# psklavos1/NeRF-Sys

Hardware: AMD Instinct MI355X
Metric: rays/sec (train step) + full-image PSNR, 800×800 Lego, 64+128 samples (higher is better)
Workload: dtype f32; 1 GPU; Lego-style 800x800 (synthetic analytic scene, 100 views), 64 coarse + 128 fine hierarchical, 2 x (8x256 MLP), fp32, train step incl. ray gen + Adam [fused engine]; global_batch=4096, rays_per_gpu=4096, parallelism=dp1, precision=fp32, fp32_gemm=split, full=False

## Files before the change

### include/nerf_amd.h

```cpp
#ifndef NERF_AMD_H
#define NERF_AMD_H

#include <stdint.h>
#include <stddef.h>
#include <hip/hip_runtime_api.h>

#ifdef __cplusplus
extern "C" {
#endif

#define NERF_OK 0
#define NERF_E_ARG (-1)
#define NERF_E_ALIGN (-2)
#define NERF_E_ENUM (-3)
#define NERF_E_WORKSPACE (-4)
#define NERF_E_UNSUPPORTED (-5)


int nerf_rays_gen(const float* c2w, int n_poses, const int32_t* pix, int64_t n, int H, int W,
                  float fx, float fy, float cx, float cy, int center_pixels, float near_v, float far_v,
                  const float* aabb, float aabb_max_bound, float aabb_invalid,
                  const uint8_t* images_u8, float* rays_out, float* rgb_out, hipStream_t stream);

int nerf_pick_pixels(int64_t n, int n_images, int H, int W, uint64_t seed, int32_t* pix_out,
                     hipStream_t stream);

int nerf_pick_pixels_dseed(int64_t n, int n_images, int H, int W, uint64_t seed_base, uint64_t seed_mul,
                           const int64_t* step_dev, int32_t* pix_out, hipStream_t stream);

int nerf_clamp_near_far(float* rays, int64_t n, int has_near, float near_v, int has_far, float far_v,
                        float eps, float invalid_value, uint8_t* valid_out, hipStream_t stream);

int nerf_rays_ndc(const float* rays_in, int64_t n, int H, int W, float focal, float near_plane,
                  float* rays_out, hipStream_t stream);


int nerf_sample_stratified(const float* rays, int64_t n, int S, int randomized, const float* u,
                           uint64_t seed, float* t_out, hipStream_t stream);

int nerf_build_xd(const float* rays, const float* t, int64_t n, int S, float* xd_out, hipStream_t stream);

int nerf_sample_pdf(const float* t, const float* w, int64_t n, int S, int n_imp, const float* u, int det,
                    uint64_t seed, float* t_out, hipStream_t stream);


int nerf_freq_encode(const float* x, int64_t n, int D, int L, int include_input, float* out, int ld_out,
                     hipStream_t stream);


int64_t nerf_mlp_layout(int64_t* table);

int64_t nerf_mlp_workspace_bytes(int64_t M, int training);

int nerf_mlp_fwd(const float* w, const float* x_d, int64_t M, float* rgb_sigma, void* ws, int64_t ws_bytes,
                 int training, hipEvent_t* events, hipStream_t stream);


int nerf_mlp_bwd(const float* w, int64_t M, const float* d_rgb_sigma, float* d_w, int accumulate, void* ws,
                 int64_t ws_bytes, hipEvent_t* events, hipStream_t stream);

int64_t nerf_mlp_workspace_bytes_2s(int64_t M);
int nerf_mlp_bwd_2s(const float* w, int64_t M, const float* d_rgb_sigma, float* d_w, int accumulate, void* ws,
                    int64_t ws_bytes, hipEvent_t* events, hipStream_t stream, hipStream_t wgrad_stream, hipEvent_t* sync);

#define NERF_MLP_NATIVE_FP32 1
#define NERF_MLP_NATIVE_DGRAD 2
int nerf_mlp_fwd_ex(const float* w, const float* x_d, int64_t M, float* rgb_sigma, void* ws, int64_t ws_bytes,
                    int training, int flags, hipEvent_t* events, hipStream_t stream);
int nerf_mlp_bwd_ex(const float* w, int64_t M, const float* d_rgb_sigma, float* d_w, int accumulate, void* ws,
                    int64_t ws_bytes, int flags, hipEvent_t* events, hipStream_t stream);
int nerf_mlp_bwd_2s_ex(const float* w, int64_t M, const float* d_rgb_sigma, float* d_w, int accumulate, void* ws,
                       int64_t ws_bytes, int flags, hipEvent_t* events, hipStream_t stream, hipStream_t wgrad_stream,
                       hipEvent_t* sync);

#define NERF_BF16_LAYERED_FWD 1
#define NERF_BF16_LAYERED_BWD 2
int64_t nerf_mlp_workspace_bytes_bf16(int64_t M, int training);
int nerf_mlp_fwd_bf16(const float* w, const float* x_d, int64_t M, float* rgb_sigma, void* ws, int64_t ws_bytes,
                      int training, int flags, hipEvent_t* events, hipStream_t stream);
int nerf_mlp_bwd_bf16(const float* w, int64_t M, const float* d_rgb_sigma, float* d_w, int accumulate, void* ws,
                      int64_t ws_bytes, int flags, hipEvent_t* events, hipStream_t stream);

int64_t nerf_mlp_workspace_bytes_f16(int64_t M, int training);
int nerf_mlp_fwd_f16(const float* w, const float* x_d, int64_t M, float* rgb_sigma, void* ws, int64_t ws_bytes,
                     int training, int flags, hipEvent_t* events, hipStream_t stream);
int nerf_mlp_bwd_f16(const float* w, int64_t M, const float* d_rgb_sigma, float* d_w, int accumulate, void* ws,
                     int64_t ws_bytes, int flags, hipEvent_t* events, hipStream_t stream);


int nerf_composite_fwd(const float* rgb_sigma, const float* t, const float* bg, int64_t n, int S,
                       float sigma_scale, float* rgb, float* depth, float* weights, float* acc,
                       const float* gt, int color_space, float inv_count, float* loss_sum, float* d_rgb,
                       hipStream_t stream);

int nerf_composite_bwd(const float* rgb_sigma, const float* t, const float* bg, int64_t n, int S,
                       float sigma_scale, const float* g_rgb, const float* g_depth, const float* g_acc,
                       const float* g_weights, float* d_rgb_sigma, hipStream_t stream);


int nerf_grad_sqnorm(const float* g, int64_t n, float* partials, hipStream_t stream);

int nerf_adam(float* p, const float* g, float* m, float* v, int64_t n, const int64_t* seg_off_host,
              const double* seg_lr_host, int n_seg, double beta1, double beta2, float eps, float weight_decay,
              int step, const float* partials, float max_norm, hipStream_t stream);

int nerf_adam_dstep(float* p, const float* g, float* m, float* v, int64_t n, const int64_t* seg_off_host,
                    const double* seg_lr_host, int n_seg, double beta1, double beta2, float eps, float weight_decay,
                    const int64_t* step_dev, const float* partials, float max_norm, hipStream_t stream);


#define NERF_HASH_MAX_LEVELS 32

typedef struct {
  int32_t levels;
  int32_t features_per_level;
  int32_t log2_hashmap_size;
  int32_t interpolation;
  int32_t resolutions[NERF_HASH_MAX_LEVELS];
} NerfHashGrid;
// ... 194 lines not shown
```

### nerf-sys_amd/csrc/gemm_x6.hpp

```cpp
#pragma once
#include "gemm_bf16.hpp"

typedef float x6_f32x2 __attribute__((ext_vector_type(2)));
typedef __bf16 x6_bf16x2 __attribute__((ext_vector_type(2)));
typedef float x6_f32x4 __attribute__((ext_vector_type(4)));
__device__ __forceinline__ uint32_t x6_pack(float a, float b) {
  return __builtin_bit_cast(uint32_t, __builtin_convertvector(x6_f32x2{a, b}, x6_bf16x2));
}

__device__ __forceinline__ void x6_split4(const float4 v, uint2& h, uint2& m, uint2& l) {
  const uint32_t h0 = x6_pack(v.x, v.y), h1 = x6_pack(v.z, v.w);
  const float r0 = v.x - nerf_bf16_lo(h0), r1 = v.y - nerf_bf16_hi(h0);
  const float r2 = v.z - nerf_bf16_lo(h1), r3 = v.w - nerf_bf16_hi(h1);
  const uint32_t m0 = x6_pack(r0, r1), m1 = x6_pack(r2, r3);
  const uint32_t l0 = x6_pack(r0 - nerf_bf16_lo(m0), r1 - nerf_bf16_hi(m0));
  const uint32_t l1 = x6_pack(r2 - nerf_bf16_lo(m1), r3 - nerf_bf16_hi(m1));
  h = make_uint2(h0, h1);
  m = make_uint2(m0, m1);
  l = make_uint2(l0, l1);
}

__device__ constexpr int X6_PA[6] = {2, 1, 0, 1, 0, 0};
__device__ constexpr int X6_PB[6] = {0, 1, 2, 0, 1, 0};
#define X6_MFMA_BLOCK(acc_, TM_, TN_, FIRST_, SECOND_)                                                      \
  _Pragma("unroll") for (int t_ = 0; t_ < 6; ++t_)                                                        \
    _Pragma("unroll") for (int a_ = 0; a_ < TM_; ++a_)                                                    \
      _Pragma("unroll") for (int b_ = 0; b_ < TN_; ++b_)                                                  \
        acc_[a_][b_] = __builtin_amdgcn_mfma_f32_32x32x16_bf16(FIRST_, SECOND_, acc_[a_][b_], 0, 0, 0);

struct X6Job {
  const float* src;
  nerf_bf16* dst;
  int rows, cols, lds, transpose;
  int64_t plane;
};
struct X6Jobs {
  X6Job j[16];
};
static __global__ void x6_planes_kernel(X6Jobs jobs) {
  const X6Job J = jobs.j[blockIdx.z];
  __shared__ float tile[32][33];
  const int r0 = blockIdx.y * 32, c0 = blockIdx.x * 32;
  if (r0 >= J.rows || c0 >= J.cols) return;
  const int tx = threadIdx.x & 31, ty = threadIdx.x >> 5;
  for (int y = ty; y < 32; y += 8) {
    const int r = r0 + y, c = c0 + tx;
    tile[y][tx] = (r < J.rows && c < J.cols) ? J.src[(int64_t)r * J.lds + c] : 0.f;
  }
  __syncthreads();
  for (int y = ty; y < 32; y += 8) {
    const float v = J.transpose ? tile[tx][y] : tile[y][tx];
    const int orow = J.transpose ? c0 + y : r0 + y, ocol = J.transpose ? r0 + tx : c0 + tx;
    const int orows = J.transpose ? J.cols : J.rows, ocols = J.transpose ? J.rows : J.cols;
    if (orow < orows && ocol < ocols) {
      const nerf_bf16 h = (nerf_bf16)v;
      const float r1 = v - (float)h;
      const nerf_bf16 m = (nerf_bf16)r1;
      const nerf_bf16 l = (nerf_bf16)(r1 - (float)m);
      const int64_t o = (int64_t)orow * ocols + ocol;
      J.dst[o] = h;
      J.dst[J.plane + o] = m;
      J.dst[2 * J.plane + o] = l;
    }
  }
}


constexpr int X6E_PITCH = 36;
constexpr int X6E_WAVE_FLOATS = 32 * X6E_PITCH;
template <int TM, int TN, int EPI>
__device__ __forceinline__ void x6_epilogue_lds(nerf_f32x16 (&acc)[TM][TN], int64_t mw, int n0, int lane,
                                                const float* __restrict__ bias, float* __restrict__ C, int ldc,
                                                const uint32_t* __restrict__ mbits, int ldmb,
                                                uint32_t* __restrict__ mbits_out, float* E) {
  const int li = lane & 31, lh = lane >> 5;
  const int rr = lane >> 3, cc = 4 * (lane & 7);
#pragma unroll
  for (int b = 0; b < TN; ++b) {
    const int nb = n0 + b * 32;
    const int g = nb >> 5;
    float4 bv[4];
#pragma unroll
    for (int q = 0; q < 4; ++q) {
      bv[q] = make_float4(0.f, 0.f, 0.f, 0.f);
      if (EPI == EPI_BIAS || EPI == EPI_BIAS_RELU) bv[q] = *reinterpret_cast<const float4*>(bias + nb + 8 * q + 4 * lh);
    }
#pragma unroll
    for (int a = 0; a < TM; ++a) {
      const int64_t m = mw + a * 32 + li;
      uint32_t word = 0;
      if (EPI == EPI_MASK) word = mbits[m * ldmb + g];
#pragma unroll
      for (int q = 0; q < 4; ++q) {
        float v[4];
#pragma unroll
        for (int e = 0; e < 4; ++e) {
          v[e] = acc[a][b][4 * q + e];
          const float bb = e == 0 ? bv[q].x : (e == 1 ? bv[q].y : (e == 2 ? bv[q].z : bv[q].w));
          if (EPI == EPI_BIAS) v[e] += bb;
          if (EPI == EPI_BIAS_RELU) {
            v[e] = fmaxf(v[e] + bb, 0.f);
            word |= (v[e] > 0.f ? 1u : 0u) << (8 * q + 4 * lh + e);
          }
          if (EPI == EPI_MASK) v[e] = ((word >> (8 * q + 4 * lh + e)) & 1u) ? v[e] : 0.f;
        }
        *reinterpret_cast<float4*>(E + li * X6E_PITCH + 8 * q + 4 * lh) = make_float4(v[0], v[1], v[2], v[3]);
      }
      if (EPI == EPI_BIAS_RELU && mbits_out) {
        word |= __shfl_xor(word, 32, 64);
        if (lh == 0) mbits_out[m * ldmb + g] = word;
      }
      float4 o[4];
#pragma unroll
      for (int i = 0; i < 4; ++i) o[i] = *reinterpret_cast<const float4*>(E + (rr + 8 * i) * X6E_PITCH + cc);
#pragma unroll
      for (int i = 0; i < 4; ++i)
        *reinterpret_cast<float4*>(C + (mw + a * 32 + rr + 8 * i) * ldc + nb + cc) = o[i];
    }
  }
}

template <int EPI, bool BIGSMALL, int NKC, int TN>
__global__ __launch_bounds__(512, 1) void gemm_nt_x6w_kernel(const float* __restrict__ A, int lda,
                                                             const nerf_bf16* __restrict__ Bp, int ldb, int64_t bplane,
                                                             const float* __restrict__ bias, float* __restrict__ C,
                                                             int ldc, const uint32_t* __restrict__ mbits, int ldmb,
                                                             uint32_t* __restrict__ mbits_out, int K, int n_ntiles) {
  constexpr int BK = 32, NW = 8, TM = 1;
  constexpr int WTM = 32 * TM, BM = WTM * NW, BN = 32 * TN;
  constexpr int KS = BK / 16;
  constexpr int LS = BK;
  static_assert(BK == 32, "the swizzle assumes four 16-B chunks per row");
  auto sw = [](int r, int q) { return q ^ ((r >> 2) & 3); };
  constexpr int PL = BN * LS;
  static_assert(2 * 3 * PL >= NW * X6E_WAVE_FLOATS * 2, "epilogue tiles");
  __shared__ __attribute__((aligned(16))) nerf_bf16 smem[2 * 3 * PL];

  const int tile = xcd_remap(blockIdx.x, gridDim.x);
  const int mt = tile / n_ntiles, nt = tile - mt * n_ntiles;
  const int64_t m0 = (int64_t)mt * BM;
  const int n0 = nt * BN;
  const int tid = threadIdx.x, lane = tid & 63, wave = tid >> 6;
  const int li = lane & 31, lh = lane >> 5;
  const nerf_bf16* Bb = Bp + (int64_t)n0 * ldb;
  const float* At = A + (m0 + wave * WTM) * lda;
  int aoff[TM];
#pragma unroll
  for (int a = 0; a < TM; ++a) aoff[a] = (a * 32 + li) * lda + 8 * lh;

  constexpr bool A3 = NKC > 0;
  float4 ra[A3 ? 3 : 2][TM][KS][2];
  constexpr int GPP = BN * BK * 2 / 1024, GPW = 3 * GPP / NW;
  static_assert(GPW * NW == 3 * GPP && GPP * 1024 == BN * BK * 2, "weight staging");
  const int wave_u = __builtin_amdgcn_readfirstlane(tid >> 6);
  const uint32_t gofs = (uint32_t)((((lane >> 2) * ldb) + 8 * ((lane & 3) ^ ((lane >> 4) & 3))) * 2);
  const uint32_t smem_u32 = (uint32_t)(uintptr_t)(const __attribute__((address_space(3))) char*)smem;
#define X6W_ALOAD(set_, k0_)                                                                              \
  _Pragma("unroll") for (int a = 0; a < TM; ++a)                                                         \
    _Pragma("unroll") for (int ks = 0; ks < KS; ++ks)                                                    \
      _Pragma("unroll") for (int hf = 0; hf < 2; ++hf)                                                   \
        ra[set_][a][ks][hf] = *reinterpret_cast<const float4*>(At + aoff[a] + (k0_) + 16 * ks + 4 * hf);
  constexpr int BPG = 2;
#define X6W_BLOAD(k0_, dbuf_)                                                                             \
  {                                                                                                       \
    _Pragma("unroll") for (int a = 0; a < TM; ++a)                                                       \
      _Pragma("unroll") for (int ks = 0; ks < KS; ++ks)                                                  \
        asm volatile("" ::"v"(__builtin_bit_cast(x6_f32x4, ra[j][a][ks][0])),                            \
                     "v"(__builtin_bit_cast(x6_f32x4, ra[j][a][ks][1])) : "memory");                     \
    _Pragma("unroll") for (int i = 0; i < GPW; ++i) {                                                    \
      const int g_ = wave_u + NW * i, p_ = g_ / GPP, rb_ = (g_ % GPP) * 16;                              \
      const nerf_bf16* sb_ = Bb + p_ * bplane + (int64_t)rb_ * ldb + (k0_);                              \
      const uint32_t dst_ = smem_u32 + (uint32_t)((((dbuf_) * 3 + p_) * PL + rb_ * LS) * 2);             \
      unsigned keep_;                                                                                     \
      asm volatile("s_mov_b32 %0, m0\n\ts_mov_b32 m0, %3\n\ts_nop 0\n\tglobal_load_lds_dwordx4 %1, %2\n\t" \
                   "s_mov_b32 m0, %0" : "=&s"(keep_) : "v"(gofs), "s"(sb_), "s"(dst_) : "memory");       \
    }                                                                                                     \
  }
  static_assert(TM * KS * 2 == 4, "vmcnt: the activation loads after the weight DMA");
#define X6W_BWAIT() asm volatile("s_waitcnt vmcnt(4)" ::: "memory")

  nerf_f32x16 acc[TM][TN], accs[BIGSMALL ? TM : 1][BIGSMALL ? TN : 1];
#pragma unroll
  for (int a = 0; a < TM; ++a)
#pragma unroll
    for (int b = 0; b < TN; ++b)
#pragma unroll
      for (int r = 0; r < 16; ++r) {
        acc[a][b][r] = 0.f;
        if constexpr (BIGSMALL) accs[a][b][r] = 0.f;
      }

  const int nk = A3 ? NKC : K / BK;
  X6W_ALOAD(0, 0);
  X6W_ALOAD(1, (nk > 1 ? 1 : 0) * BK);
  {
    const int j = 0;
    X6W_BLOAD(0, 0);
    asm volatile("s_waitcnt vmcnt(0)" ::: "memory");
  }
  __syncthreads();
  auto slab_mfma = [&](const float4 (&rj)[TM][KS][2], const nerf_bf16* S, auto&& after_split) __attribute__((always_inline)) {
#pragma unroll
        for (int ks = 0; ks < KS; ++ks) {
          nerf_bf16x8 af[TM][3];
#pragma unroll
          for (int a = 0; a < TM; ++a) {
            uint2 h0, m0_, l0, h1, m1, l1;
            x6_split4(rj[a][ks][0], h0, m0_, l0);
            x6_split4(rj[a][ks][1], h1, m1, l1);
            af[a][0] = __builtin_bit_cast(nerf_bf16x8, make_uint4(h0.x, h0.y, h1.x, h1.y));
            af[a][1] = __builtin_bit_cast(nerf_bf16x8, make_uint4(m0_.x, m0_.y, m1.x, m1.y));
            af[a][2] = __builtin_bit_cast(nerf_bf16x8, make_uint4(l0.x, l0.y, l1.x, l1.y));
          }
          if (ks == KS - 1) after_split();
#pragma unroll
          for (int bp = 0; bp < TN / BPG; ++bp) {
            nerf_bf16x8 bf[BPG][3];
#pragma unroll
            for (int p = 0; p < 3; ++p)
#pragma unroll
              for (int b = 0; b < BPG; ++b)
                bf[b][p] = *reinterpret_cast<const nerf_bf16x8*>(S + p * PL + ((BPG * bp + b) * 32 + li) * LS +
                                                                 8 * sw((BPG * bp + b) * 32 + li, 2 * ks + lh));
#pragma unroll
            for (int t = 0; t < 6; ++t)
#pragma unroll
              for (int a = 0; a < TM; ++a)
#pragma unroll
                for (int b = 0; b < BPG; ++b) {
                  if constexpr (BIGSMALL) {
                    if (t < 5)
                      accs[a][BPG * bp + b] = __builtin_amdgcn_mfma_f32_32x32x16_bf16(
                          bf[b][X6_PB[t]], af[a][X6_PA[t]], accs[a][BPG * bp + b], 0, 0, 0);
                    else
                      acc[a][BPG * bp + b] = __builtin_amdgcn_mfma_f32_32x32x16_bf16(
                          bf[b][X6_PB[t]], af[a][X6_PA[t]], acc[a][BPG * bp + b], 0, 0, 0);
                  } else {
                    acc[a][BPG * bp + b] = __builtin_amdgcn_mfma_f32_32x32x16_bf16(
                        bf[b][X6_PB[t]], af[a][X6_PA[t]], acc[a][BPG * bp + b], 0, 0, 0);
                  }
                }
          }
        }
  };
  if constexpr (A3) {
#pragma unroll
    for (int kt = 0; kt < NKC; ++kt) {
      const int j = kt % 3;
      X6W_BLOAD((kt + 1 < NKC ? kt + 1 : kt) * BK, (kt + 1) & 1);
      if (kt + 2 < NKC) X6W_ALOAD((kt + 2) % 3, (kt + 2) * BK);
      asm volatile("" ::: "memory");
      slab_mfma(ra[j], smem + (kt & 1) * 3 * PL, [] {});
      if (kt + 2 < NKC) {
        X6W_BWAIT();
      } else {
        asm volatile("s_waitcnt vmcnt(0)" ::: "memory");
      }
      __syncthreads();
    }
  } else {
    for (int kt0 = 0; kt0 < nk; kt0 += 2) {
#pragma unroll
      for (int j = 0; j < 2; ++j) {
        const int kt = kt0 + j;
        X6W_BLOAD((kt + 1 < nk ? kt + 1 : kt) * BK, j ^ 1);
        slab_mfma(ra[j], smem + j * 3 * PL, [&] {
          X6W_ALOAD(j, (kt + 2 < nk ? kt + 2 : nk - 1) * BK);
          asm volatile("" ::: "memory");
        });
        X6W_BWAIT();
        __syncthreads();
      }
    }
    asm volatile("s_waitcnt vmcnt(0)" ::: "memory");
    __syncthreads();
  }
#undef X6W_ALOAD
#undef X6W_BLOAD
#undef X6W_BWAIT

  if constexpr (BIGSMALL) {
#pragma unroll
    for (int a = 0; a < TM; ++a)
#pragma unroll
      for (int b = 0; b < TN; ++b) acc[a][b] += accs[a][b];
  }
  x6_epilogue_lds<TM, TN, EPI>(acc, m0 + wave * WTM, n0, lane, bias, C, ldc, mbits, ldmb, mbits_out,
                               reinterpret_cast<float*>(smem) + wave * X6E_WAVE_FLOATS);
}

template <int BN, int BK, int WAVES_N>
__global__ __launch_bounds__(256, 2) void gemm_wgrad_x6_kernel(const float* __restrict__ G, int ldg,
                                                              const float* __restrict__ X, int ldx,
                                                              float* __restrict__ P, int ldp, float* __restrict__ Pb,
                                                              int64_t slab, int64_t rows_per_split, int64_t M,
                                                              int n_ktiles, int n_tiles) {
  constexpr int MR = 16;
  constexpr int WAVES_K = 4 / WAVES_N;
  constexpr int WTN = BN / WAVES_N, WTK = BK / WAVES_K;
  constexpr int TM = WTN / 32, TN = WTK / 32;
  static_assert(TM >= 1 && TN >= 1, "wave tile");
  constexpr int PG = ((BN + 127) / 128) * 128 + 32, PX = ((BK + 127) / 128) * 128 + 32;
  constexpr int IG = MR * PG, IX = MR * PX;
  constexpr int STAGE = 3 * (IG + IX);
  constexpr int G_F4 = MR * BN / 4, X_F4 = MR * BK / 4;
  constexpr int G_PER = (G_F4 + 255) / 256, X_PER = (X_F4 + 255) / 256;
  __shared__ __attribute__((aligned(16))) nerf_bf16 smem[2 * STAGE];

  const int lin = xcd_remap(blockIdx.x, gridDim.x);
  const int s = lin / n_tiles;
  const int tile = lin - s * n_tiles;
  const int nt = tile / n_ktiles, kt = tile - nt * n_ktiles;
  const int n0 = nt * BN, k0 = kt * BK;
  const int64_t r0 = (int64_t)s * rows_per_split;
  int64_t r1 = r0 + rows_per_split;
  if (r1 > M) r1 = M;
  const int tid = threadIdx.x, lane = tid & 63, wave = tid >> 6;
  const int wn = wave / WAVES_K, wk = wave % WAVES_K;
  const int li = lane & 31, lh = lane >> 5;
  const bool do_bias = (Pb != nullptr) && kt == 0 && wk == 0;

  constexpr int PF = 4;
  float4 rg[PF][G_PER], rx[PF][X_PER];
#define WX6_GLOAD(set_, m_)                                                                                \
  {                                                                                                        \
    _Pragma("unroll") for (int i = 0; i < G_PER; ++i) {                                                    \
      const int f = tid + 256 * i;                                                                         \
      if (G_F4 % 256 == 0 || f < G_F4)                                                                     \
        rg[set_][i] = *reinterpret_cast<const float4*>(G + ((m_) + f / (BN / 4)) * ldg + n0 + (f % (BN / 4)) * 4); \
    }                                                                                                      \
    _Pragma("unroll") for (int i = 0; i < X_PER; ++i) {                                                    \
      const int f = tid + 256 * i;                                                                         \
      if (X_F4 % 256 == 0 || f < X_F4)                                                                     \
        rx[set_][i] = *reinterpret_cast<const float4*>(X + ((m_) + f / (BK / 4)) * ldx + k0 + (f % (BK / 4)) * 4); \
    }                                                                                                      \
  }
#define WX6_SSTORE(set_, buf_)                                                                             \
  {                                                                                                        \
    nerf_bf16* Gs_ = smem + (buf_) * STAGE;                                                                \
    nerf_bf16* Xs_ = Gs_ + 3 * IG;                                                                         \
    _Pragma("unroll") for (int i = 0; i < G_PER; ++i) {                                                    \
// ... 267 lines not shown
```

### nerf-sys_amd/csrc/mlp.hip

```cpp
#include "gemm.hpp"
#include "gemm_x6.hpp"
#include "mlp_common.hpp"
#include "mlp_tail.hpp"
#include "mlp_fwd_tail.hpp"

namespace {
using namespace nerf_mlp;

struct WS {
  int64_t Mp;
  float *X3E, *Y[8], *HO, *CIN, *C0;
  uint32_t* MB[8];
  float *dA, *dB, *dO16, *WT, *partial, *partial2;
  float* dZ[8];
  nerf_bf16* WPf;
  nerf_bf16* WPb;
  int S;
  int64_t rps;
  int64_t bytes;
};

constexpr int64_t WT_FLOATS = 7 * 65536;
inline int64_t x6_fwd_off(int i) {
  int64_t o = 0;
// ... 179 lines not shown
  }
  return NERF_OK;
}

int wgrad_x6(const float* G, int ldg, const float* X, int ldx, int tensor_w, const WS& w, int N, int K, hipStream_t st) {
  const Layout& L = layout();
  float* P = w.partial + L.off[tensor_w];
  float* Pb = w.partial + L.off[tensor_w + 1];
  const int ldp = L.cols[tensor_w];
  const int64_t slab = L.total;
  if (N != 256 || ldg % 4 || ldx % 4) return NERF_E_ARG;
  auto t128 = [&](const float* Xk, float* Pk, float* Pbk) {
    gemm_wgrad_x6w_kernel<<<w.S, 512, 0, st>>>(G, ldg, Xk, ldx, Pk, ldp, Pbk, slab, w.rps, w.Mp);
  };
  auto t64 = [&](const float* Xk, float* Pk, float* Pbk) {
    gemm_wgrad_x6_kernel<128, 64, 4><<<2 * w.S, 256, 0, st>>>(G, ldg, Xk, ldx, Pk, ldp, Pbk, slab, w.rps, w.Mp, 1, 2);
  };
  if (K == 64) {
    t64(X, P, Pb);
  } else if (K == 256) {
    t128(X, P, Pb);
  } else if (K == 320) {
    t128(X, P, Pb);
    t64(X + 256, P + 256, nullptr);
  } else {
    return NERF_E_ARG;
  }
  return NERF_OK;
}

}

extern "C" int64_t nerf_mlp_layout(int64_t* table) {
  const Layout& L = layout();
  if (table) {
    for (int t = 0; t < NT; ++t) {
      table[4 * t + 0] = L.off[t];
      table[4 * t + 1] = L.rows[t];
      table[4 * t + 2] = L.cols[t];
      table[4 * t + 3] = L.creal[t];
    }
  }
  return L.total;
}

extern "C" int64_t nerf_mlp_workspace_bytes(int64_t M, int training) {
  if (M < 0) return -1;
  return carve(nullptr, M, training).bytes + 256;
}

extern "C" int nerf_mlp_fwd_ex(const float* w, const float* x_d, int64_t M, float* rgb_sigma, void* ws,
                               int64_t ws_bytes, int training, int flags, hipEvent_t* ev, hipStream_t st) {
  NERF_CHECK_ARG(w && ws && M >= 0 && (M == 0 || (x_d && rgb_sigma)));
  if (flags & ~NERF_MLP_NATIVE_FP32) return NERF_E_ENUM;
  const bool native = flags & NERF_MLP_NATIVE_FP32;
  if (!nerf_aligned16(w) || !nerf_aligned16(ws) || !nerf_aligned16(rgb_sigma)) return NERF_E_ALIGN;
  const WS W = carve(ws, M, training);
  if (ws_bytes < W.bytes) return NERF_E_WORKSPACE;
  if (M == 0) return NERF_OK;
  const Layout& L = layout();
  const int64_t Mp = W.Mp;
  auto Wt = [&](int t) { return w + L.off[t]; };

  pe_xyz_kernel<<<(unsigned)nerf_cdiv(Mp, 256), 256, 0, st>>>(x_d, M, Mp, W.X3E);
  if (!native) {
    X6Jobs jobs{};
    for (int i = 0; i < 8; ++i)
      jobs.j[i] = X6Job{Wt(2 * i), W.WPf + x6_fwd_off(i), 256, KPAD[i], KPAD[i], 0, 256 * (int64_t)KPAD[i]};
    x6_planes_kernel<<<dim3(10, 8, 8), 256, 0, st>>>(jobs);
  }
  const float* in = W.X3E + 256;
  int ld_in = 320;
  for (int i = 0; i < 8; ++i) {
    float* out = W.Y[i];
    const int ld_out = training ? ld_of(W, i) : ((i % 2 == 0) ? 256 : 320);
    if (i == 4) { in = W.X3E; ld_in = 320; }
    if (ev) (void)hipEventRecord(ev[2 * i], st);
    if (native)
      TRY(nt<EPI_BIAS_RELU>(in, ld_in, Wt(2 * i), KPAD[i], Wt(2 * i + 1), out, ld_out, nullptr,
                            training ? W.MB[i] : nullptr, Mp, 256, KPAD[i], st));
    else
      TRY(nt_x6<EPI_BIAS_RELU>(in, ld_in, W.WPf + x6_fwd_off(i), KPAD[i], 256 * (int64_t)KPAD[i], Wt(2 * i + 1), out,
                               ld_out, nullptr, training ? W.MB[i] : nullptr, Mp, 256, KPAD[i], st));
    if (ev) (void)hipEventRecord(ev[2 * i + 1], st);
    in = out;
    ld_in = ld_out;
  }
  {
    FwdTailArgs T{};
    T.Y7 = in; T.ldy = ld_in; T.xd = x_d; T.w = w;
    T.off_wh = L.off[16]; T.off_bh = L.off[17]; T.off_wc0 = L.off[18]; T.off_bc0 = L.off[19];
    T.off_wc1 = L.off[20]; T.off_bc1 = L.off[21];
    T.HO = W.HO; T.CIN = W.CIN; T.C0 = W.C0; T.out = rgb_sigma;
    T.M = M; T.Mp = Mp; T.ntiles = (int)(Mp / FT_ROWS);
    const int n_cu = nerf_cu_count();
    const int grid = T.ntiles < 2 * n_cu ? T.ntiles : 2 * n_cu;
    if (training)
      fwd_tail_kernel<true><<<grid, 256, 0, st>>>(T);
    else
      fwd_tail_kernel<false><<<grid, 256, 0, st>>>(T);
  }
  return nerf_launch_status();
}


extern "C" int nerf_mlp_fwd(const float* w, const float* x_d, int64_t M, float* rgb_sigma, void* ws, int64_t ws_bytes,
                            int training, hipEvent_t* ev, hipStream_t st) {
  return nerf_mlp_fwd_ex(w, x_d, M, rgb_sigma, ws, ws_bytes, training, 0, ev, st);
}

extern "C" int64_t nerf_mlp_workspace_bytes_2s(int64_t M) {
  if (M < 0) return -1;
  return carve(nullptr, M, 2).bytes + 256;
}

namespace {
int mlp_bwd_impl(const float* w, int64_t M, const float* d_rgb_sigma, float* d_w, int accumulate, void* ws,
                 int64_t ws_bytes, int flags, hipEvent_t* ev, hipStream_t st, hipStream_t stw, hipEvent_t* sync) {
  NERF_CHECK_ARG(w && d_w && ws && M >= 0 && (M == 0 || d_rgb_sigma));
  NERF_CHECK_ARG(!stw || sync);
  if (flags & ~(NERF_MLP_NATIVE_FP32 | NERF_MLP_NATIVE_DGRAD)) return NERF_E_ENUM;
  const bool native = flags & NERF_MLP_NATIVE_FP32;
  const bool split_dgrad = !native && !(flags & NERF_MLP_NATIVE_DGRAD);
  if (!nerf_aligned16(w) || !nerf_aligned16(ws) || !nerf_aligned16(d_w) || !nerf_aligned16(d_rgb_sigma))
    return NERF_E_ALIGN;
  const bool two = stw != nullptr;
  const WS W = carve(ws, M, two ? 2 : 1);
  if (ws_bytes < W.bytes) return NERF_E_WORKSPACE;
  hipStream_t sw = two ? stw : st;
  auto handoff = [&](int k) -> int {
    if (!two) return NERF_OK;
    hipError_t e = hipEventRecord(sync[k], st);
    if (e == hipSuccess) e = hipStreamWaitEvent(stw, sync[k], 0);
    return nerf_hip_status(e);
  };
  const Layout& L = layout();
  if (M == 0) {
    if (!accumulate) (void)hipMemsetAsync(d_w, 0, L.total * sizeof(float), st);
    return nerf_launch_status();
// ... 88 lines not shown
```

### nerf-sys_amd/nerf_amd/kernels.py

```python
from __future__ import annotations

import ctypes
from typing import Sequence

import torch

from ._lib import check, lib, need, ptr, stream

F32 = torch.float32
_CS = {"linear": 0, "srgb": 1, "identity": 2}


def _empty(shape, like):
    return torch.empty(shape, dtype=F32, device=like.device)


def rays_gen(c2w, H, W, fx, fy, cx, cy, *, pix=None, near=None, far=None, aabb=None, center_pixels=True,
             images_u8=None, aabb_max_bound=1e10, aabb_invalid=1e10):
    need(c2w, "c2w")
    if c2w.dim() == 2:
        c2w = c2w[:3, :4].reshape(1, 3, 4).contiguous()
    c2w = c2w[..., :3, :4].contiguous()
    n_poses = c2w.shape[0]
    if pix is not None:
# ... 74 lines not shown
    check(lib().nerf_sample_pdf(ptr(t), ptr(w), n, S, n_imp, ptr(u), int(bool(det)),
                                ctypes.c_uint64(seed & (2**64 - 1)), ptr(out), stream()), "nerf_sample_pdf")
    return out


def freq_encode(x, L, include_input=True):
    need(x, "x")
    D = x.shape[-1]
    flat = x.reshape(-1, D)
    od = D * (2 * L + (1 if include_input else 0))
    out = _empty((flat.shape[0], od), x)
    check(lib().nerf_freq_encode(ptr(flat), flat.shape[0], D, L, int(include_input), ptr(out), od, stream()),
          "nerf_freq_encode")
    return out.view(*x.shape[:-1], od)




PRECISIONS = ("fp32", "bf16", "fp16")
_H16 = {"bf16": "bf16", "fp16": "f16"}
BF16_LAYERED_FWD = 1
BF16_LAYERED_BWD = 2


def _check_precision(precision):
    if precision not in PRECISIONS:
        raise ValueError(f"precision must be one of {PRECISIONS}, got {precision!r}")


def mlp_workspace_bytes(M, training, precision="fp32"):
    _check_precision(precision)
    if precision in _H16:
        return getattr(lib(), f"nerf_mlp_workspace_bytes_{_H16[precision]}")(M, int(training))
    return lib().nerf_mlp_workspace_bytes(M, int(training))


def mlp_workspace_bytes_2s(M):
    return lib().nerf_mlp_workspace_bytes_2s(M)


def mlp_workspace(M, training, device, precision="fp32"):
    return torch.empty(mlp_workspace_bytes(M, training, precision), dtype=torch.uint8, device=device)


def _events_arg(events):
    if events is None:
        return None
    arr = (ctypes.c_void_p * len(events))(*[ctypes.c_void_p(e.cuda_event) for e in events])
    return arr


MLP_NATIVE_FP32 = 1
MLP_NATIVE_DGRAD = 2


def mlp_fwd(w_packed, x_d, ws, training, out=None, events=None, precision="fp32", bf16_flags=0, fp32_flags=0):
    need(w_packed, "packed weights"), need(x_d, "x_d")
    _check_precision(precision)
    M = x_d.shape[0]
    if out is None:
        out = _empty((M, 4), x_d)
    if precision in _H16:
        fn = f"nerf_mlp_fwd_{_H16[precision]}"
        check(getattr(lib(), fn)(ptr(w_packed), ptr(x_d), M, ptr(out), ptr(ws), ws.numel(), int(training),
                                 int(bf16_flags), _events_arg(events), stream()), fn)
        return out
    check(lib().nerf_mlp_fwd_ex(ptr(w_packed), ptr(x_d), M, ptr(out), ptr(ws), ws.numel(), int(training),
                                int(fp32_flags) & MLP_NATIVE_FP32,
                                _events_arg(events), stream()), "nerf_mlp_fwd_ex")
    return out


def mlp_bwd(w_packed, M, d_rgb_sigma, ws, d_w=None, accumulate=False, events=None, precision="fp32", bf16_flags=0,
            wgrad_stream=None, sync=None, fp32_flags=0):
    need(w_packed, "packed weights"), need(d_rgb_sigma, "d_rgb_sigma")
    _check_precision(precision)
    if d_w is None:
        d_w = torch.empty_like(w_packed)
        accumulate = False
    if precision in _H16:
        fn = f"nerf_mlp_bwd_{_H16[precision]}"
        check(getattr(lib(), fn)(ptr(w_packed), M, ptr(d_rgb_sigma), ptr(d_w), int(accumulate), ptr(ws),
                                 ws.numel(), int(bf16_flags), _events_arg(events), stream()), fn)
        return d_w
    if wgrad_stream is not None:
        if sync is None or len(sync) < 10:
            raise ValueError("nerf_mlp_bwd_2s needs 10 sync events")
        for e in sync:
            if not e.cuda_event:
                e.record()
        check(lib().nerf_mlp_bwd_2s_ex(ptr(w_packed), M, ptr(d_rgb_sigma), ptr(d_w), int(accumulate), ptr(ws),
                                       ws.numel(), int(fp32_flags), _events_arg(events), stream(),
                                       ctypes.c_void_p(wgrad_stream.cuda_stream), _events_arg(sync)),
              "nerf_mlp_bwd_2s_ex")
        return d_w
    check(lib().nerf_mlp_bwd_ex(ptr(w_packed), M, ptr(d_rgb_sigma), ptr(d_w), int(accumulate), ptr(ws), ws.numel(),
                                int(fp32_flags), _events_arg(events), stream()), "nerf_mlp_bwd_ex")
    return d_w




def composite_fwd(rgb_sigma, t, bg=None, sigma_scale=1.0, gt=None, color_space="linear", inv_count=None,
                  loss_sum=None, outs=None):
    need(rgb_sigma, "rgb_sigma"), need(t, "t")
    n, S = t.shape
    if bg is not None:
        need(bg, "bg")
    if outs is None:
        rgb, depth, w, acc = _empty((n, 3), t), _empty((n,), t), _empty((n, S), t), _empty((n,), t)
    else:
        rgb, depth, w, acc = outs
    d_rgb = None
    if gt is not None:
        need(gt, "gt")
        d_rgb = _empty((n, 3), t)
        if loss_sum is None:
            loss_sum = torch.zeros(1, dtype=F32, device=t.device)
        if inv_count is None:
            inv_count = 1.0 / (3 * n)
    cs = _CS.get(color_space)
    if cs is None:
        raise ValueError(f"Invalid color_space={color_space!r}; use 'linear'|'srgb'|'identity'")
    check(lib().nerf_composite_fwd(ptr(rgb_sigma), ptr(t), ptr(bg), n, S, float(sigma_scale), ptr(rgb), ptr(depth),
                                   ptr(w), ptr(acc), ptr(gt), cs, float(inv_count or 0.0), ptr(loss_sum),
                                   ptr(d_rgb), stream()), "nerf_composite_fwd")
    if gt is not None:
        return rgb, depth, w, acc, loss_sum, d_rgb
    return rgb, depth, w, acc


def composite_bwd(rgb_sigma, t, bg, g_rgb, g_depth=None, g_acc=None, g_w=None, sigma_scale=1.0, out=None):
    need(rgb_sigma, "rgb_sigma"), need(t, "t"), need(g_rgb, "g_rgb")
    n, S = t.shape
    if rgb_sigma.numel() != n * S * 4 or rgb_sigma.shape[-1] != 4:
        raise ValueError(f"rgb_sigma must hold ({n},{S},4), got {tuple(rgb_sigma.shape)}")
    if tuple(g_rgb.shape) != (n, 3):
        raise ValueError(f"g_rgb must be ({n},3), got {tuple(g_rgb.shape)}")
    for x, name, shape in ((bg, "bg", (n, 3)), (g_depth, "g_depth", (n,)), (g_acc, "g_acc", (n,)),
                           (g_w, "g_w", (n, S))):
        if x is not None:
            need(x, name)
            if tuple(x.shape) != shape:
                raise ValueError(f"{name} must be {shape}, got {tuple(x.shape)}")
    if out is None:
        out = torch.empty_like(rgb_sigma)
    else:
        need(out, "out")
    check(lib().nerf_composite_bwd(ptr(rgb_sigma), ptr(t), ptr(bg), n, S, float(sigma_scale), ptr(g_rgb),
                                   ptr(g_depth), ptr(g_acc), ptr(g_w), ptr(out), stream()), "nerf_composite_bwd")
# ... 33 lines not shown
```

Measured before the change: 251,800 rays/s.

## Chain the eight forward MLP layers into one persistent fp32-split GEMM kernel

Adds a chained kernel in which each 256-row block runs all eight forward trunk layers back to back. It hands the next layer's activations through registers using permlane32 swaps instead of reloading them, and prefetches the next layer's weights during the last k-slab. Bias rows are staged in LDS. This is meant to remove seven launches and the per-layer global reload of activations. In exchange it keeps one block per 256 rows, which lowers parallelism, and adds synchronisation between layers; the old per-layer path stays behind a new FWD_LAYERED flag.

```diff
diff --git a/include/nerf_amd.h b/include/nerf_amd.h
--- a/include/nerf_amd.h
+++ b/include/nerf_amd.h
@@ -65,6 +65,7 @@
 
 #define NERF_MLP_NATIVE_FP32 1
 #define NERF_MLP_NATIVE_DGRAD 2
+#define NERF_MLP_FWD_LAYERED 4
 int nerf_mlp_fwd_ex(const float* w, const float* x_d, int64_t M, float* rgb_sigma, void* ws, int64_t ws_bytes,
                     int training, int flags, hipEvent_t* events, hipStream_t stream);
 int nerf_mlp_bwd_ex(const float* w, int64_t M, const float* d_rgb_sigma, float* d_w, int accumulate, void* ws,
diff --git a/nerf-sys_amd/csrc/gemm_x6.hpp b/nerf-sys_amd/csrc/gemm_x6.hpp
--- a/nerf-sys_amd/csrc/gemm_x6.hpp
+++ b/nerf-sys_amd/csrc/gemm_x6.hpp
@@ -68,11 +68,22 @@
 
 constexpr int X6E_PITCH = 36;
 constexpr int X6E_WAVE_FLOATS = 32 * X6E_PITCH;
-template <int TM, int TN, int EPI>
+__device__ __forceinline__ void x6_swap32(float& a, float& b) {
+  typedef unsigned x6_u32x2 __attribute__((ext_vector_type(2)));
+  const x6_u32x2 r = __builtin_amdgcn_permlane32_swap(__builtin_bit_cast(unsigned, a), __builtin_bit_cast(unsigned, b),
+                                                      false, false);
+  const unsigned r0 = r[0], r1 = r[1];
+  a = __builtin_bit_cast(float, r0);
+  b = __builtin_bit_cast(float, r1);
+}
+
+template <int TM, int TN, int EPI, bool HAND = false>
 __device__ __forceinline__ void x6_epilogue_lds(nerf_f32x16 (&acc)[TM][TN], int64_t mw, int n0, int lane,
                                                 const float* __restrict__ bias, float* __restrict__ C, int ldc,
                                                 const uint32_t* __restrict__ mbits, int ldmb,
-                                                uint32_t* __restrict__ mbits_out, float* E) {
+                                                uint32_t* __restrict__ mbits_out, float* E,
+                                                float4 (*ho)[1][2][2] = nullptr, const float* bias_lds = nullptr) {
+  static_assert(!HAND || (TM == 1 && TN >= 2 && EPI == EPI_BIAS_RELU), "hand-off: the forward tile");
   const int li = lane & 31, lh = lane >> 5;
   const int rr = lane >> 3, cc = 4 * (lane & 7);
 #pragma unroll
@@ -83,13 +94,18 @@
 #pragma unroll
     for (int q = 0; q < 4; ++q) {
       bv[q] = make_float4(0.f, 0.f, 0.f, 0.f);
-      if (EPI == EPI_BIAS || EPI == EPI_BIAS_RELU) bv[q] = *reinterpret_cast<const float4*>(bias + nb + 8 * q + 4 * lh);
+      if constexpr (HAND) {
+        bv[q] = *reinterpret_cast<const float4*>(bias_lds + nb + 8 * q + 4 * lh);
+      } else if (EPI == EPI_BIAS || EPI == EPI_BIAS_RELU) {
+        bv[q] = *reinterpret_cast<const float4*>(bias + nb + 8 * q + 4 * lh);
+      }
     }
 #pragma unroll
     for (int a = 0; a < TM; ++a) {
       const int64_t m = mw + a * 32 + li;
       uint32_t word = 0;
       if (EPI == EPI_MASK) word = mbits[m * ldmb + g];
+      float hv[4][4];
 #pragma unroll
       for (int q = 0; q < 4; ++q) {
         float v[4];
@@ -103,8 +119,25 @@
             word |= (v[e] > 0.f ? 1u : 0u) << (8 * q + 4 * lh + e);
           }
           if (EPI == EPI_MASK) v[e] = ((word >> (8 * q + 4 * lh + e)) & 1u) ? v[e] : 0.f;
+          if constexpr (HAND) hv[q][e] = v[e];
         }
         *reinterpret_cast<float4*>(E + li * X6E_PITCH + 8 * q + 4 * lh) = make_float4(v[0], v[1], v[2], v[3]);
+      }
+      if constexpr (HAND) {
+        if (b < 2) {
+#pragma unroll
+          for (int ks = 0; ks < 2; ++ks) {
+            float f0[4], f1[4];
+#pragma unroll
+            for (int e = 0; e < 4; ++e) {
+              f0[e] = hv[2 * ks][e];
+              f1[e] = hv[2 * ks + 1][e];
+              x6_swap32(f0[e], f1[e]);
+            }
+            ho[b][0][ks][0] = make_float4(f0[0], f0[1], f0[2], f0[3]);
+            ho[b][0][ks][1] = make_float4(f1[0], f1[1], f1[2], f1[3]);
+          }
+        }
       }
       if (EPI == EPI_BIAS_RELU && mbits_out) {
         word |= __shfl_xor(word, 32, 64);
@@ -120,12 +153,18 @@
   }
 }
 
-template <int EPI, bool BIGSMALL, int NKC, int TN>
-__global__ __launch_bounds__(512, 1) void gemm_nt_x6w_kernel(const float* __restrict__ A, int lda,
-                                                             const nerf_bf16* __restrict__ Bp, int ldb, int64_t bplane,
-                                                             const float* __restrict__ bias, float* __restrict__ C,
-                                                             int ldc, const uint32_t* __restrict__ mbits, int ldmb,
-                                                             uint32_t* __restrict__ mbits_out, int K, int n_ntiles) {
+template <int TN>
+constexpr int x6w_smem_elems() { return 2 * 3 * (32 * TN) * 32; }
+
+template <int EPI, bool BIGSMALL, int NKC, int TN, int CH = 0>
+__device__ __forceinline__ void x6w_tile(const float* __restrict__ A, int lda, const nerf_bf16* __restrict__ Bp,
+                                         int ldb, int64_t bplane, const float* __restrict__ bias,
+                                         float* __restrict__ C, int ldc, const uint32_t* __restrict__ mbits, int ldmb,
+                                         uint32_t* __restrict__ mbits_out, int K, int64_t m0, int n0,
+                                         nerf_bf16* smem, float4 (&ra)[NKC > 0 ? 3 : 2][1][2][2],
+                                         const nerf_bf16* nBp = nullptr, int nldb = 0, int64_t nbplane = 0,
+                                         bool first = true) {
+  static_assert(CH == 0 || (NKC == 0 && EPI == EPI_BIAS_RELU), "chained: the forward tile");
   constexpr int BK = 32, NW = 8, TM = 1;
   constexpr int WTM = 32 * TM, BM = WTM * NW, BN = 32 * TN;
   constexpr int KS = BK / 16;
@@ -134,12 +173,10 @@
   auto sw = [](int r, int q) { return q ^ ((r >> 2) & 3); };
   constexpr int PL = BN * LS;
   static_assert(2 * 3 * PL >= NW * X6E_WAVE_FLOATS * 2, "epilogue tiles");
-  __shared__ __attribute__((aligned(16))) nerf_bf16 smem[2 * 3 * PL];
-
-  const int tile = xcd_remap(blockIdx.x, gridDim.x);
-  const int mt = tile / n_ntiles, nt = tile - mt * n_ntiles;
-  const int64_t m0 = (int64_t)mt * BM;
-  const int n0 = nt * BN;
+  static_assert(CH == 0 || 3 * PL >= NW * (X6E_WAVE_FLOATS + BN) * 2, "epilogue tiles and bias rows in buffer 1");
+  static_assert(CH == 0 || BN == 256, "bias row: one float4 per lane");
+  static_assert(2 * 3 * PL == x6w_smem_elems<TN>(), "weight buffers");
+
   const int tid = threadIdx.x, lane = tid & 63, wave = tid >> 6;
   const int li = lane & 31, lh = lane >> 5;
   const nerf_bf16* Bb = Bp + (int64_t)n0 * ldb;
@@ -149,11 +186,12 @@
   for (int a = 0; a < TM; ++a) aoff[a] = (a * 32 + li) * lda + 8 * lh;
 
   constexpr bool A3 = NKC > 0;
-  float4 ra[A3 ? 3 : 2][TM][KS][2];
   constexpr int GPP = BN * BK * 2 / 1024, GPW = 3 * GPP / NW;
   static_assert(GPW * NW == 3 * GPP && GPP * 1024 == BN * BK * 2, "weight staging");
   const int wave_u = __builtin_amdgcn_readfirstlane(tid >> 6);
   const uint32_t gofs = (uint32_t)((((lane >> 2) * ldb) + 8 * ((lane & 3) ^ ((lane >> 4) & 3))) * 2);
+  const uint32_t ngofs = (uint32_t)((((lane >> 2) * nldb) + 8 * ((lane & 3) ^ ((lane >> 4) & 3))) * 2);
+  const nerf_bf16* nBb = nBp + (int64_t)n0 * nldb;
   const uint32_t smem_u32 = (uint32_t)(uintptr_t)(const __attribute__((address_space(3))) char*)smem;
 #define X6W_ALOAD(set_, k0_)                                                                              \
   _Pragma("unroll") for (int a = 0; a < TM; ++a)                                                         \
@@ -161,7 +199,8 @@
       _Pragma("unroll") for (int hf = 0; hf < 2; ++hf)                                                   \
         ra[set_][a][ks][hf] = *reinterpret_cast<const float4*>(At + aoff[a] + (k0_) + 16 * ks + 4 * hf);
   constexpr int BPG = 2;
-#define X6W_BLOAD(k0_, dbuf_)                                                                             \
+#define X6W_BLOAD(k0_, dbuf_) X6W_BLOAD_SRC(Bb, ldb, bplane, gofs, k0_, dbuf_)
+#define X6W_BLOAD_SRC(Bb_, ldb_, bplane_, gofs_, k0_, dbuf_)                                              \
   {                                                                                                       \
     _Pragma("unroll") for (int a = 0; a < TM; ++a)                                                       \
       _Pragma("unroll") for (int ks = 0; ks < KS; ++ks)                                                  \
@@ -169,11 +208,11 @@
                      "v"(__builtin_bit_cast(x6_f32x4, ra[j][a][ks][1])) : "memory");                     \
     _Pragma("unroll") for (int i = 0; i < GPW; ++i) {                                                    \
       const int g_ = wave_u + NW * i, p_ = g_ / GPP, rb_ = (g_ % GPP) * 16;                              \
-      const nerf_bf16* sb_ = Bb + p_ * bplane + (int64_t)rb_ * ldb + (k0_);                              \
+      const nerf_bf16* sb_ = (Bb_) + p_ * (bplane_) + (int64_t)rb_ * (ldb_) + (k0_);                     \
       const uint32_t dst_ = smem_u32 + (uint32_t)((((dbuf_) * 3 + p_) * PL + rb_ * LS) * 2);             \
       unsigned keep_;                                                                                     \
       asm volatile("s_mov_b32 %0, m0\n\ts_mov_b32 m0, %3\n\ts_nop 0\n\tglobal_load_lds_dwordx4 %1, %2\n\t" \
-                   "s_mov_b32 m0, %0" : "=&s"(keep_) : "v"(gofs), "s"(sb_), "s"(dst_) : "memory");       \
+                   "s_mov_b32 m0, %0" : "=&s"(keep_) : "v"(gofs_), "s"(sb_), "s"(dst_) : "memory");      \
     }                                                                                                     \
   }
   static_assert(TM * KS * 2 == 4, "vmcnt: the activation loads after the weight DMA");
@@ -191,14 +230,18 @@
       }
 
   const int nk = A3 ? NKC : K / BK;
-  X6W_ALOAD(0, 0);
-  X6W_ALOAD(1, (nk > 1 ? 1 : 0) * BK);
-  {
-    const int j = 0;
-    X6W_BLOAD(0, 0);
-    asm volatile("s_waitcnt vmcnt(0)" ::: "memory");
-  }
-  __syncthreads();
+  float4 bz = make_float4(0.f, 0.f, 0.f, 0.f);
+  if constexpr (CH != 0) bz = *reinterpret_cast<const float4*>(bias + n0 + 4 * lane);
+  if (CH == 0 || first) {
+    X6W_ALOAD(0, 0);
+    X6W_ALOAD(1, (nk > 1 ? 1 : 0) * BK);
+    {
+      const int j = 0;
+      X6W_BLOAD(0, 0);
+      asm volatile("s_waitcnt vmcnt(0)" ::: "memory");
+    }
+    __syncthreads();
+  }
   auto slab_mfma = [&](const float4 (&rj)[TM][KS][2], const nerf_bf16* S, auto&& after_split) __attribute__((always_inline)) {
 #pragma unroll
         for (int ks = 0; ks < KS; ++ks) {
@@ -211,6 +254,12 @@
             af[a][0] = __builtin_bit_cast(nerf_bf16x8, make_uint4(h0.x, h0.y, h1.x, h1.y));
             af[a][1] = __builtin_bit_cast(nerf_bf16x8, make_uint4(m0_.x, m0_.y, m1.x, m1.y));
             af[a][2] = __builtin_bit_cast(nerf_bf16x8, make_uint4(l0.x, l0.y, l1.x, l1.y));
+          }
+          if constexpr (CH != 0) {
+            if (ks == KS - 1) {
+#pragma unroll
+              for (int a = 0; a < TM; ++a) asm volatile("" ::"v"(af[a][0]), "v"(af[a][1]), "v"(af[a][2]) : "memory");
+            }
           }
           if (ks == KS - 1) after_split();
 #pragma unroll
@@ -263,7 +312,13 @@
 #pragma unroll
       for (int j = 0; j < 2; ++j) {
         const int kt = kt0 + j;
-        X6W_BLOAD((kt + 1 < nk ? kt + 1 : kt) * BK, j ^ 1);
+        if (CH != 0 && j == 1) {
+          const bool nx = nBp != nullptr && kt + 1 >= nk;
+          X6W_BLOAD_SRC((nx ? nBb : Bb), (nx ? nldb : ldb), (nx ? nbplane : bplane), (nx ? ngofs : gofs),
+                        (nx ? 0 : (kt + 1 < nk ? kt + 1 : kt) * BK), j ^ 1);
+        } else {
+          X6W_BLOAD((kt + 1 < nk ? kt + 1 : kt) * BK, j ^ 1);
+        }
         slab_mfma(ra[j], smem + j * 3 * PL, [&] {
           X6W_ALOAD(j, (kt + 2 < nk ? kt + 2 : nk - 1) * BK);
           asm volatile("" ::: "memory");
@@ -277,6 +332,7 @@
   }
 #undef X6W_ALOAD
 #undef X6W_BLOAD
+#undef X6W_BLOAD_SRC
 #undef X6W_BWAIT
 
   if constexpr (BIGSMALL) {
@@ -285,8 +341,62 @@
 #pragma unroll
       for (int b = 0; b < TN; ++b) acc[a][b] += accs[a][b];
   }
-  x6_epilogue_lds<TM, TN, EPI>(acc, m0 + wave * WTM, n0, lane, bias, C, ldc, mbits, ldmb, mbits_out,
-                               reinterpret_cast<float*>(smem) + wave * X6E_WAVE_FLOATS);
+  float* Eb = nullptr;
+  if constexpr (CH != 0) {
+    Eb = reinterpret_cast<float*>(smem + 3 * PL) + NW * X6E_WAVE_FLOATS + wave * BN - n0;
+    *reinterpret_cast<float4*>(Eb + n0 + 4 * lane) = bz;
+  }
+  x6_epilogue_lds<TM, TN, EPI, CH != 0>(acc, m0 + wave * WTM, n0, lane, bias, C, ldc, mbits, ldmb, mbits_out,
+                                        reinterpret_cast<float*>(smem + (CH != 0 ? 3 * PL : 0)) + wave * X6E_WAVE_FLOATS,
+                                        CH != 0 ? &ra[0] : nullptr, Eb);
+}
+
+template <int EPI, bool BIGSMALL, int NKC, int TN>
+__global__ __launch_bounds__(512, 1) void gemm_nt_x6w_kernel(const float* __restrict__ A, int lda,
+                                                             const nerf_bf16* __restrict__ Bp, int ldb, int64_t bplane,
+                                                             const float* __restrict__ bias, float* __restrict__ C,
+                                                             int ldc, const uint32_t* __restrict__ mbits, int ldmb,
+                                                             uint32_t* __restrict__ mbits_out, int K, int n_ntiles) {
+  __shared__ __attribute__((aligned(16))) nerf_bf16 smem[x6w_smem_elems<TN>()];
+  const int tile = xcd_remap(blockIdx.x, gridDim.x);
+  const int mt = tile / n_ntiles, nt = tile - mt * n_ntiles;
+  float4 ra[NKC > 0 ? 3 : 2][1][2][2];
+  x6w_tile<EPI, BIGSMALL, NKC, TN>(A, lda, Bp, ldb, bplane, bias, C, ldc, mbits, ldmb, mbits_out, K, (int64_t)mt * 256,
+                                   nt * 32 * TN, smem, ra);
+}
+
+struct X6ChainLayer {
+  const float* A;
+  const nerf_bf16* Bp;
+  const float* bias;
+  float* C;
+  uint32_t* mbits_out;
+  int64_t bplane;
+  int lda, ldb, ldc, K;
+};
+constexpr int X6_CHAIN_MAX = 8;
+struct X6Chain {
+  X6ChainLayer l[X6_CHAIN_MAX];
+  int n;
+};
+__global__ __launch_bounds__(512, 1) void gemm_nt_x6w_chain_kernel(const X6Chain ch) {
+  __shared__ __attribute__((aligned(16))) nerf_bf16 smem[x6w_smem_elems<8>()];
+  const int64_t m0 = (int64_t)xcd_remap(blockIdx.x, gridDim.x) * 256;
+  float4 ra[2][1][2][2];
+#define X6_CHAIN_NEXT()                                        \
+  __builtin_amdgcn_fence(__ATOMIC_RELEASE, "wavefront");       \
+  __builtin_amdgcn_fence(__ATOMIC_ACQUIRE, "wavefront");       \
+  __syncthreads();
+#pragma unroll 1
+  for (int i = 0; i < ch.n; ++i) {
+    const X6ChainLayer& L = ch.l[i];
+    const X6ChainLayer& N = ch.l[i + 1 < ch.n ? i + 1 : i];
+    x6w_tile<EPI_BIAS_RELU, false, 0, 8, 1>(L.A, L.lda, L.Bp, L.ldb, L.bplane, L.bias, L.C, L.ldc, nullptr, 8,
+                                            L.mbits_out, L.K, m0, 0, smem, ra, i + 1 < ch.n ? N.Bp : nullptr, N.ldb,
+                                            N.bplane, i == 0);
+    X6_CHAIN_NEXT()
+  }
+#undef X6_CHAIN_NEXT
 }
 
 template <int BN, int BK, int WAVES_N>
diff --git a/nerf-sys_amd/csrc/mlp.hip b/nerf-sys_amd/csrc/mlp.hip
--- a/nerf-sys_amd/csrc/mlp.hip
+++ b/nerf-sys_amd/csrc/mlp.hip
@@ -255,8 +255,9 @@
 extern "C" int nerf_mlp_fwd_ex(const float* w, const float* x_d, int64_t M, float* rgb_sigma, void* ws,
                                int64_t ws_bytes, int training, int flags, hipEvent_t* ev, hipStream_t st) {
   NERF_CHECK_ARG(w && ws && M >= 0 && (M == 0 || (x_d && rgb_sigma)));
-  if (flags & ~NERF_MLP_NATIVE_FP32) return NERF_E_ENUM;
+  if (flags & ~(NERF_MLP_NATIVE_FP32 | NERF_MLP_FWD_LAYERED)) return NERF_E_ENUM;
   const bool native = flags & NERF_MLP_NATIVE_FP32;
+  const bool chained = !native && !ev && !(flags & NERF_MLP_FWD_LAYERED);
   if (!nerf_aligned16(w) || !nerf_aligned16(ws) || !nerf_aligned16(rgb_sigma)) return NERF_E_ALIGN;
   const WS W = carve(ws, M, training);
   if (ws_bytes < W.bytes) return NERF_E_WORKSPACE;
@@ -274,10 +275,18 @@
   }
   const float* in = W.X3E + 256;
   int ld_in = 320;
+  X6Chain chain{};
   for (int i = 0; i < 8; ++i) {
     float* out = W.Y[i];
     const int ld_out = training ? ld_of(W, i) : ((i % 2 == 0) ? 256 : 320);
     if (i == 4) { in = W.X3E; ld_in = 320; }
+    if (chained) {
+      chain.l[i] = X6ChainLayer{in, W.WPf + x6_fwd_off(i), Wt(2 * i + 1), out, training ? W.MB[i] : nullptr,
+                                256 * (int64_t)KPAD[i], ld_in, KPAD[i], ld_out, KPAD[i]};
+      in = out;
+      ld_in = ld_out;
+      continue;
+    }
     if (ev) (void)hipEventRecord(ev[2 * i], st);
     if (native)
       TRY(nt<EPI_BIAS_RELU>(in, ld_in, Wt(2 * i), KPAD[i], Wt(2 * i + 1), out, ld_out, nullptr,
@@ -288,6 +297,14 @@
     if (ev) (void)hipEventRecord(ev[2 * i + 1], st);
     in = out;
     ld_in = ld_out;
+  }
+  if (chained) {
+    chain.n = 8;
+    for (int i = 0; i < 8; ++i) {
+      if (chain.l[i].K % 64 || chain.l[i].lda % 4 || chain.l[i].ldb % 8) return NERF_E_ARG;
+      if (i > 0 && (chain.l[i].A != chain.l[i - 1].C || chain.l[i].lda != chain.l[i - 1].ldc)) return NERF_E_ARG;
+    }
+    gemm_nt_x6w_chain_kernel<<<(unsigned)(Mp / 256), 512, 0, st>>>(chain);
   }
   {
     FwdTailArgs T{};
diff --git a/nerf-sys_amd/nerf_amd/kernels.py b/nerf-sys_amd/nerf_amd/kernels.py
--- a/nerf-sys_amd/nerf_amd/kernels.py
+++ b/nerf-sys_amd/nerf_amd/kernels.py
@@ -150,6 +150,7 @@
 
 MLP_NATIVE_FP32 = 1
 MLP_NATIVE_DGRAD = 2
+MLP_FWD_LAYERED = 4
 
 
 def mlp_fwd(w_packed, x_d, ws, training, out=None, events=None, precision="fp32", bf16_flags=0, fp32_flags=0):
@@ -164,7 +165,7 @@
                                  int(bf16_flags), _events_arg(events), stream()), fn)
         return out
     check(lib().nerf_mlp_fwd_ex(ptr(w_packed), ptr(x_d), M, ptr(out), ptr(ws), ws.numel(), int(training),
-                                int(fp32_flags) & MLP_NATIVE_FP32,
+                                int(fp32_flags) & ~MLP_NATIVE_DGRAD,
                                 _events_arg(events), stream()), "nerf_mlp_fwd_ex")
     return out
 
@@ -188,12 +189,13 @@
             if not e.cuda_event:
                 e.record()
         check(lib().nerf_mlp_bwd_2s_ex(ptr(w_packed), M, ptr(d_rgb_sigma), ptr(d_w), int(accumulate), ptr(ws),
-                                       ws.numel(), int(fp32_flags), _events_arg(events), stream(),
+                                       ws.numel(), int(fp32_flags) & ~MLP_FWD_LAYERED, _events_arg(events), stream(),
                                        ctypes.c_void_p(wgrad_stream.cuda_stream), _events_arg(sync)),
               "nerf_mlp_bwd_2s_ex")
         return d_w
     check(lib().nerf_mlp_bwd_ex(ptr(w_packed), M, ptr(d_rgb_sigma), ptr(d_w), int(accumulate), ptr(ws), ws.numel(),
-                                int(fp32_flags), _events_arg(events), stream()), "nerf_mlp_bwd_ex")
+                                int(fp32_flags) & ~MLP_FWD_LAYERED,
+                                _events_arg(events), stream()), "nerf_mlp_bwd_ex")
     return d_w
 
 
```

Measured after the change: 261,300 rays/s, median of 6. +3.7%, better.
